# TWeber132/thesis-clip-nerf

Hardware: AMD Instinct MI355X
Metric: rendered rays/sec (64 samples/ray) at 1/2/4/8 MI355X; RGB L1 vs ref (higher is better)
Workload: dtype f32

## Files before the change

### thesis_clip_nerf_amd/csrc/field_eval_split16_impl.h

```cpp
#include <hip/hip_runtime.h>

#include "mvnerf_kernels.h"
#include "mvnerf_launch.h"
#include "mvnerf_math.h"
#include "mvnerf_mfma.h"

#ifndef MVS16_F16
#error "include through field_eval_split16.hip / field_eval_split16h.hip"
#endif
#if MVS16_F16
#define MVS16_BYTES packed_net_split16h_bytes
#define MVS16_PACK launch_pack_net_split16h
#define MVS16_SUPPORTS field_eval_split16h_supports
#define MVS16_LAUNCH_FN launch_field_eval_split16h
#define MVS16_KERNEL field_eval_split16h_kernel
#define MVS16_PACK_KERNEL pack_net_split16h_kernel
#else
#define MVS16_BYTES packed_net_split16_bytes
#define MVS16_PACK launch_pack_net_split16
#define MVS16_SUPPORTS field_eval_split16_supports
#define MVS16_LAUNCH_FN launch_field_eval_split16
#define MVS16_KERNEL field_eval_split16_kernel
#define MVS16_PACK_KERNEL pack_net_split16_kernel
#endif

namespace mvnerf {

namespace {

using bf16x8 = __attribute__((ext_vector_type(8))) __bf16;
using f16x8 = __attribute__((ext_vector_type(8))) _Float16;
using f16x2 = __attribute__((ext_vector_type(2))) _Float16;
using f32x2 = __attribute__((ext_vector_type(2))) float;
using u32x4 = __attribute__((ext_vector_type(4))) unsigned int;

constexpr int kS16SlotChunks = 24;
constexpr int kS16L0Pe = 2, kS16L0Feat = 8, kS16Hidden = 48;
constexpr int kS16Steps = kS16L0Pe + kS16L0Feat + kS16Hidden;
constexpr int kS16Chunks = kS16Steps * kS16SlotChunks;
constexpr int kChunkElems16 = 512;

__host__ __device__ constexpr int s16_pe_row(int g, int e) {
    return g < 3 ? 20 * g + e : (e < 12 ? 20 * (e >> 2) + 2 * (8 + ((e >> 1) & 1)) + (e & 1) : (e < 15 ? 120 + (e - 12) : -1));
}

__global__ void MVS16_PACK_KERNEL(const float* __restrict__ src, unsigned short* __restrict__ dst) {
    const int idx = blockIdx.x * blockDim.x + threadIdx.x;
    if (idx >= kS16Chunks * kChunkElems16) return;
    const int chunk = idx / kChunkElems16, lane = (idx % kChunkElems16) / 8, jj = idx % 8;
    const int i = lane & 15, g = lane >> 4;
    const int ks = chunk / kS16SlotChunks, rb = (chunk % kS16SlotChunks) / 3, piece = chunk % 3;
    float val = 0.0f;
    if (ks < kS16L0Pe) {
        const int row = s16_pe_row(g, 8 * ks + jj);
        if (row >= 0) val = src[kKerasW0 + row * kHidden + 16 * rb + i];
    } else if (ks < kS16L0Pe + kS16L0Feat) {
        const int row = 123 + 32 * (ks - kS16L0Pe) + 8 * g + jj;
        val = src[kKerasW0 + row * kHidden + 16 * rb + i];
    } else {
        const int q = ks - kS16L0Pe - kS16L0Feat, layer = q / 4, t = q % 4;
        const int f = 32 * t + (jj < 4 ? 4 * g + jj : 16 + 4 * g + (jj - 4));
        const int wsrc = kKerasBlocks + (layer / 2) * kKerasBlockStride + (layer % 2) * (kHidden * kHidden + kHidden);
        val = src[wsrc + f * kHidden + 16 * rb + i];
    }
#if MVS16_F16
    const float tw = val * 64.0f;
    const _Float16 a0 = (_Float16)tw;
    const _Float16 a1 = (_Float16)(tw - (float)a0);
    const _Float16 a0s = (_Float16)((float)a0 * 0.015625f);
    const _Float16 pc = piece == 0 ? a0 : (piece == 1 ? a0s : a1);
    dst[idx] = __builtin_bit_cast(unsigned short, pc);
#else
    const __bf16 p1 = (__bf16)val;
    const float r1 = val - (float)p1;
    const __bf16 p2 = (__bf16)r1;
    const float r2 = r1 - (float)p2;
    const __bf16 p3 = (__bf16)r2;
    const __bf16 pc = piece == 0 ? p1 : (piece == 1 ? p2 : p3);
    dst[idx] = __builtin_bit_cast(unsigned short, pc);
#endif
}

__device__ __forceinline__ f32x4 mfma1632(u32x4 a, u32x4 b, f32x4 c) {
#if MVS16_F16
    return __builtin_amdgcn_mfma_f32_16x16x32_f16(__builtin_bit_cast(f16x8, a), __builtin_bit_cast(f16x8, b), c, 0, 0, 0);
#else
    return __builtin_amdgcn_mfma_f32_16x16x32_bf16(__builtin_bit_cast(bf16x8, a), __builtin_bit_cast(bf16x8, b), c, 0, 0, 0);
#endif
}

struct B16 {
    u32x4 p1, p2, p3;
};

template <bool kRelu>
__device__ __forceinline__ void cut_pair(float v0, float v1, int q, B16& b) {
    if (kRelu) {
        const int i0 = __builtin_bit_cast(int, v0), i1 = __builtin_bit_cast(int, v1);
        v0 = __builtin_bit_cast(float, i0 > 0 ? i0 : 0);
        v1 = __builtin_bit_cast(float, i1 > 0 ? i1 : 0);
    }
#if MVS16_F16
    const f32x2 t = {v0 * 0.015625f, v1 * 0.015625f};
    const unsigned h = __builtin_bit_cast(unsigned, __builtin_convertvector(t, f16x2));
    float r0, r1;
    asm("v_fma_mix_f32 %0, %1, %2, %3 op_sel_hi:[1,0,0]" : "=v"(r0) : "v"(h), "s"(-64.0f), "v"(v0));
    asm("v_fma_mix_f32 %0, %1, %2, %3 op_sel:[1,0,0] op_sel_hi:[1,0,0]" : "=v"(r1) : "v"(h), "s"(-64.0f), "v"(v1));
    const f32x2 r = {r0, r1};
    b.p1[q] = h;
    b.p3[q] = __builtin_bit_cast(unsigned, __builtin_convertvector(r, f16x2));
#else
    const float r0 = v0 - __builtin_bit_cast(float, __builtin_bit_cast(unsigned, v0) & 0xffff0000u);
    const float r1 = v1 - __builtin_bit_cast(float, __builtin_bit_cast(unsigned, v1) & 0xffff0000u);
    const float s0 = r0 - __builtin_bit_cast(float, __builtin_bit_cast(unsigned, r0) & 0xffff0000u);
    const float s1 = r1 - __builtin_bit_cast(float, __builtin_bit_cast(unsigned, r1) & 0xffff0000u);
    b.p1[q] = __builtin_amdgcn_perm(__builtin_bit_cast(unsigned, v1), __builtin_bit_cast(unsigned, v0), 0x07060302u);
    b.p2[q] = __builtin_amdgcn_perm(__builtin_bit_cast(unsigned, r1), __builtin_bit_cast(unsigned, r0), 0x07060302u);
    b.p3[q] = __builtin_amdgcn_perm(__builtin_bit_cast(unsigned, s1), __builtin_bit_cast(unsigned, s0), 0x07060302u);
#endif
}

__device__ __forceinline__ void pin_pieces(B16& b, int q) {
#if MVS16_F16
    unsigned u1 = b.p1[q], u3 = b.p3[q];
    asm volatile("" : "+v"(u1), "+v"(u3));
    b.p1[q] = u1;
    b.p3[q] = u3;
#else
    unsigned u1 = b.p1[q], u2 = b.p2[q], u3 = b.p3[q];
    asm volatile("" : "+v"(u1), "+v"(u2), "+v"(u3));
    b.p1[q] = u1;
    b.p2[q] = u2;
    b.p3[q] = u3;
#endif
}

template <bool kRelu>
__device__ __forceinline__ void cut8(const float (&v)[8], B16& b) {
#pragma unroll
    for (int q = 0; q < 4; ++q) cut_pair<kRelu>(v[2 * q], v[2 * q + 1], q, b);
}

constexpr int kR16Slots = 3, kR16SlotF4 = kS16SlotChunks * 64;
constexpr int kS16PerView = kS16Hidden / 2;
constexpr int kS16MaxPositions = 512;

struct Ring16 {
    const f32x4* w;
    f32x4* base;
    int c;
    int p, P;
    const int* table;
    int start_pf;
    int tid, wave;
    u32x4 a0[3];
};

__device__ __forceinline__ int ring16_start_chunk(int p, int V, int l0_units) {
    const int per_view = l0_units + kS16PerView;
    if (p < per_view * V) {
        const int q = p % per_view;
        return (q < kS16L0Pe ? q : (q < l0_units ? q : kS16L0Pe + kS16L0Feat + (q - l0_units))) * kS16SlotChunks;
    }
    return (kS16L0Pe + kS16L0Feat + kS16PerView + (p - per_view * V)) * kS16SlotChunks;
}

__device__ __forceinline__ void ring16_dma(const Ring16& r, int start_chunk, int slot) {
    const f32x4* src = r.w + (long)start_chunk * 64 + r.tid;
    f32x4* dst = r.base + slot * kR16SlotF4 + 64 * r.wave;
#pragma unroll
    for (int i = 0; i < 3; ++i)
        __builtin_amdgcn_global_load_lds((const __attribute__((address_space(1))) void*)(src + 512 * i),
                                         (__attribute__((address_space(3))) void*)(dst + 512 * i), 16, 0, 0);
}

__device__ __forceinline__ void ring16_fetch(Ring16& r) {
    int slot = r.c + 2;
    slot = slot >= kR16Slots ? slot - kR16Slots : slot;
    ring16_dma(r, r.start_pf, slot);
    int pp = r.p + 3;
    pp = pp >= r.P ? pp - r.P : pp;
    r.start_pf = r.table[pp];
}

__device__ __forceinline__ const f32x4* ring16_cur(const Ring16& r) { return r.base + r.c * kR16SlotF4; }
__device__ __forceinline__ const f32x4* ring16_nxt(const Ring16& r) { return r.base + (r.c + 1 == kR16Slots ? 0 : r.c + 1) * kR16SlotF4; }

__device__ __forceinline__ void ring16_next(Ring16& r) {
    asm volatile("s_waitcnt vmcnt(0) lgkmcnt(0)\n\ts_barrier" ::: "memory");
    r.c = r.c + 1 == kR16Slots ? 0 : r.c + 1;
    r.p = r.p + 1 == r.P ? 0 : r.p + 1;
}

__device__ __forceinline__ int perm_f4(int rb, int g) {
    return ((g & 1) * 64 + (rb >> 1) * 16 + 4 * (2 * (rb & 1) + (g >> 1))) >> 2;
}

template <bool kAdd>
__device__ __forceinline__ void apply_bias_row(f32x4 (&row)[2], const f32x4& bv) {
#pragma unroll
    for (int cb = 0; cb < 2; ++cb)
#pragma unroll
        for (int c = 0; c < 4; ++c) {
            if (kAdd) {
                float r = row[cb][c];
                asm("v_add_f32_e32 %0, %1, %2" : "=v"(r) : "v"(r), "v"(bv[c]));
                row[cb][c] = r;
            } else {
                row[cb][c] = bv[c];
            }
        }
}

template <bool kRelu, int kMode, bool kTailAdd>
__device__ __forceinline__ void kstep16(Ring16& ring, int lane, int g, const B16 (&b)[2], const float (&nv)[2][8], B16 (&bn)[2], f32x4 (&acc)[8][2],
                                        f32x4 (&in)[8][2], const float* __restrict__ tail_bias) {
    const f32x4* cur = ring16_cur(ring) + lane;
    const f32x4* nxt = ring16_nxt(ring) + lane;
    u32x4 a[3] = {ring.a0[0], ring.a0[1], ring.a0[2]};
    f32x4 bv = {0.0f, 0.0f, 0.0f, 0.0f};
    int glane = (g & 1) * 16 + (g >> 1);
    if (kMode == 4) asm volatile("" : "+v"(glane));
    const f32x4* tail_rows = reinterpret_cast<const f32x4*>(tail_bias) + glane;
#pragma unroll
    for (int rb = 0; rb < 8; ++rb) {
        u32x4 an[3];
#pragma unroll
        for (int q = 0; q < 3; ++q) an[q] = __builtin_bit_cast(u32x4, rb < 7 ? cur[((rb + 1) * 3 + q) * 64] : nxt[q * 64]);
        if (kMode == 1) cut_pair<kRelu>(nv[rb >> 2][2 * (rb & 3)], nv[rb >> 2][2 * (rb & 3) + 1], rb & 3, bn[rb >> 2]);
        if (kMode == 4 && tail_bias) {
            const f32x4 bv_new = tail_rows[(rb >> 1) * 4 + 2 * (rb & 1)];
            if (rb > 0) apply_bias_row<kTailAdd>(in[rb - 1], bv);
            bv = bv_new;
        }
#if MVS16_F16
#pragma unroll
        for (int cb = 0; cb < 2; ++cb) acc[rb][cb] = mfma1632(a[1], b[cb].p3, acc[rb][cb]);
#pragma unroll
        for (int cb = 0; cb < 2; ++cb) acc[rb][cb] = mfma1632(a[2], b[cb].p1, acc[rb][cb]);
#pragma unroll
        for (int cb = 0; cb < 2; ++cb) acc[rb][cb] = mfma1632(a[0], b[cb].p1, acc[rb][cb]);
#else
#pragma unroll
        for (int cb = 0; cb < 2; ++cb) acc[rb][cb] = mfma1632(a[2], b[cb].p1, acc[rb][cb]);
#pragma unroll
        for (int cb = 0; cb < 2; ++cb) acc[rb][cb] = mfma1632(a[1], b[cb].p2, acc[rb][cb]);
#pragma unroll
        for (int cb = 0; cb < 2; ++cb) acc[rb][cb] = mfma1632(a[0], b[cb].p3, acc[rb][cb]);
#pragma unroll
        for (int cb = 0; cb < 2; ++cb) acc[rb][cb] = mfma1632(a[1], b[cb].p1, acc[rb][cb]);
#pragma unroll
        for (int cb = 0; cb < 2; ++cb) acc[rb][cb] = mfma1632(a[0], b[cb].p2, acc[rb][cb]);
#pragma unroll
        for (int cb = 0; cb < 2; ++cb) acc[rb][cb] = mfma1632(a[0], b[cb].p1, acc[rb][cb]);
#endif
        __builtin_amdgcn_sched_group_barrier(0x008, 1, 0);
        __builtin_amdgcn_sched_group_barrier(0x100, kMode == 4 ? 4 : 3, 0);
#pragma unroll
        for (int m = 0; m < (MVS16_F16 ? 5 : 11); ++m) {
            if (kMode == 1) __builtin_amdgcn_sched_group_barrier(0x002, MVS16_F16 ? 2 : 1, 0);
            if (kMode == 4) __builtin_amdgcn_sched_group_barrier(0x002, MVS16_F16 ? 2 : 1, 0);
            __builtin_amdgcn_sched_group_barrier(0x008, 1, 0);
        }
        if (kMode == 1) __builtin_amdgcn_sched_group_barrier(0x002, MVS16_F16 ? 3 : 2, 0);
        __builtin_amdgcn_sched_barrier(0);
        if (rb == 0) {
            ring16_fetch(ring);
            __builtin_amdgcn_sched_barrier(0);
        }
#pragma unroll
        for (int q = 0; q < 3; ++q) a[q] = an[q];
    }
#pragma unroll
    for (int q = 0; q < 3; ++q) ring.a0[q] = a[q];
    if (kMode == 4 && tail_bias) apply_bias_row<kTailAdd>(in[7], bv);
    if (kMode == 1) {
#pragma unroll
        for (int cb = 0; cb < 2; ++cb)
#pragma unroll
            for (int q = 0; q < 4; ++q) {
                pin_pieces(bn[cb], q);
            }
    }
}

__device__ __forceinline__ void first_operand_s16(const f32x4 (&in)[8][2], B16 (&b)[2]) {
#pragma unroll
    for (int cb = 0; cb < 2; ++cb) {
        const float v8[8] = {in[0][cb][0], in[0][cb][1], in[0][cb][2], in[0][cb][3], in[1][cb][0], in[1][cb][1], in[1][cb][2], in[1][cb][3]};
        cut8<true>(v8, b[cb]);
    }
}

template <bool kTailAdd>
__device__ __forceinline__ void dense128_s16_plain(Ring16& ring, int lane, int g, f32x4 (&in)[8][2], f32x4 (&acc)[8][2], const float* __restrict__ tail_bias) {
    B16 b[2], bn[2];
    first_operand_s16(in, b);
#pragma unroll
    for (int t = 0; t < 4; ++t) {
        float nv[2][8];
#pragma unroll
        for (int cb = 0; cb < 2; ++cb)
#pragma unroll
            for (int q = 0; q < 8; ++q) nv[cb][q] = t < 3 ? in[2 * (t + 1) + (q >> 2)][cb][q & 3] : 0.0f;
        if (t < 3) kstep16<true, 1, false>(ring, lane, g, b, nv, bn, acc, in, nullptr);
        else kstep16<true, 4, kTailAdd>(ring, lane, g, b, nv, bn, acc, in, tail_bias);
        b[0] = bn[0];
        b[1] = bn[1];
        ring16_next(ring);
    }
}

template <bool kAdd>
__device__ __forceinline__ void bias16(const float* __restrict__ bperm, int g, f32x4 (&acc)[8][2]) {
    const f32x4* p = reinterpret_cast<const f32x4*>(bperm);
#pragma unroll
    for (int rb = 0; rb < 8; ++rb) {
        const f32x4 v = p[perm_f4(rb, g)];
#pragma unroll
        for (int cb = 0; cb < 2; ++cb)
#pragma unroll
            for (int c = 0; c < 4; ++c) {
                if (kAdd) {
                    float r = acc[rb][cb][c];
                    asm("v_add_f32_e32 %0, %1, %2" : "=v"(r) : "v"(r), "v"(v[c]));
                    acc[rb][cb][c] = r;
                } else {
                    acc[rb][cb][c] = v[c];
                }
            }
    }
}

constexpr int kS16StageRowBytes = 256;

__device__ __forceinline__ void store_tl16(float* __restrict__ base, long tile, int n, int g, const f32x4 (&x)[8][2]) {
    const __amdgpu_buffer_rsrc_t rsrc = __builtin_amdgcn_make_buffer_rsrc(base, 0, 0xFFFFFFFF, 0x00020000);
    const int voff = (4 * g * 32 + n) * 4;
    const int tile_off = (int)((unsigned)tile * 16384u);
#pragma unroll
    for (int rb = 0; rb < 8; ++rb)
#pragma unroll
        for (int i = 0; i < 4; ++i)
#pragma unroll
            for (int cb = 0; cb < 2; ++cb) {
                const float val = x[rb][cb][i];
                __builtin_amdgcn_raw_buffer_store_b32(__builtin_bit_cast(unsigned int, val), rsrc, voff + (i * 32 + 16 * cb) * 4,
                                                      tile_off + rb * 2048, kStashAux);
            }
}

struct SampleGeo {
    long g;
    int ray, sidx, b;
    float wx, wy, wz;
    bool valid;
};

template <bool kMultiView, bool kProj, bool kAux, bool kStash>
__global__ __launch_bounds__(512, 2) void MVS16_KERNEL(FieldParams p, const f32x4* __restrict__ wsplit) {
    constexpr int kW = 8;
    extern __shared__ __attribute__((aligned(16))) unsigned char smem_s16[];
    constexpr int kRingBytes = kR16Slots * kR16SlotF4 * 16;
    const int tid = threadIdx.x, lane = tid & 63, n = lane & 15, g = lane >> 4;
    const int wave = __builtin_amdgcn_readfirstlane(tid >> 6);
    unsigned char* stage = smem_s16 + kRingBytes + wave * (32 * kS16StageRowBytes);
    float* net = reinterpret_cast<float*>(smem_s16 + kRingBytes + kW * 32 * kS16StageRowBytes) - kPackB0;
    for (int i = tid; i < kPackBr + 8 - kPackB0; i += 64 * kW) net[kPackB0 + i] = p.net[kPackB0 + i];
    int* table = reinterpret_cast<int*>(smem_s16 + kRingBytes + kW * 32 * kS16StageRowBytes + (kPackBr + 8 - kPackB0) * 4);
    float* wr_plain = reinterpret_cast<float*>(table + kS16MaxPositions);
    for (int i = tid; i < 512; i += 64 * kW) wr_plain[i] = p.net[kPackWrPlain + i];

    Ring16 ring;
    ring.w = wsplit;
    ring.base = reinterpret_cast<f32x4*>(smem_s16);
    ring.c = 0;
    ring.p = 0;
    const int l0_units = kProj ? kS16L0Pe : kS16L0Pe + kS16L0Feat;
    ring.P = (l0_units + kS16PerView) * p.V + kS16PerView;
    for (int i = tid; i < ring.P; i += 64 * kW) table[i] = ring16_start_chunk(i, p.V, l0_units);
    ring.table = table;
    __syncthreads();
    ring.tid = tid;
    ring.wave = wave;
    ring16_dma(ring, table[0], 0);
    ring16_dma(ring, table[1], 1);
    ring.start_pf = table[2];
    asm volatile("s_waitcnt vmcnt(0)" ::: "memory");
    __syncthreads();
#pragma unroll
    for (int q = 0; q < 3; ++q) ring.a0[q] = __builtin_bit_cast(u32x4, ring16_cur(ring)[q * 64 + lane]);

    const long n_groups = (p.n_tiles + kW - 1) / kW;
    for (long grp = blockIdx.x; grp < n_groups; grp += gridDim.x) {
        long tile = grp * kW + wave;
        const bool tile_ok = tile < p.n_tiles;
        if (!tile_ok) tile = p.n_tiles - 1;
        int pS = p.S, pR = p.R, pH = p.H, pW = p.W, gl = g, nl = n;
        asm volatile("" : "+s"(pS), "+s"(pR), "+s"(pH), "+s"(pW));
        asm volatile("" : "+v"(gl), "+v"(nl));
        SampleGeo sg[2];
#pragma unroll
        for (int cb = 0; cb < 2; ++cb) {
            long gi = tile * 32 + 16 * cb + nl;
            sg[cb].valid = tile_ok && gi < p.total;
            if (gi >= p.total) gi = p.total - 1;
            sg[cb].g = gi;
            const int ray = (int)((unsigned)gi / (unsigned)pS);
            sg[cb].ray = ray;
            sg[cb].sidx = (int)gi - ray * pS;
            sg[cb].b = (int)((unsigned)ray / (unsigned)pR);
            const float ox = p.rays_o[3 * ray + 0], oy = p.rays_o[3 * ray + 1], oz = p.rays_o[3 * ray + 2];
            const float dx = p.rays_d[3 * ray + 0], dy = p.rays_d[3 * ray + 1], dz = p.rays_d[3 * ray + 2];
            const float zz = p.z[gi];
            sg[cb].wx = ox + zz * dx;
            sg[cb].wy = oy + zz * dy;
            sg[cb].wz = oz + zz * dz;
        }

        f32x4 x[8][2], hid[8][2];
        f32x4 xsum[kMultiView ? 8 : 1][2];

        const int n_views = (kMultiView || !(kAux || kStash)) ? p.V : 1;
        for (int v = 0; v < n_views; ++v) {
            int tl[2];
            float ax[2], ay[2];
            long vrow[2];
            float pe[2][16];
#pragma unroll
            for (int cb = 0; cb < 2; ++cb) {
                const int bv = sg[cb].b * p.V + v;
                const float* E = p.einv + 16 * bv;
                float cam[4];
#pragma unroll
                for (int r = 0; r < 4; ++r) cam[r] = row_dot4(E, r, sg[cb].wx, sg[cb].wy, sg[cb].wz, 1.0f);
                float pxl, pyl;
                pixel_from_cam(p.k4 + 16 * bv, cam, &pxl, &pyl);
                const Taps tp = bilinear_taps(pxl, pyl, pH, pW);
                tl[cb] = (bv * pH + tp.y0) * pW + tp.x0;
                ax[cb] = tp.ax;
                ay[cb] = tp.ay;
                vrow[cb] = ((long)bv * pR + (sg[cb].ray - sg[cb].b * pR)) * pS + sg[cb].sidx;
                if (kAux && sg[cb].valid && gl == 0) {
                    if (p.tap_idx) {
                        int4 t4 = make_int4(tl[cb], tl[cb] + 1, tl[cb] + pW, tl[cb] + pW + 1);
                        *reinterpret_cast<int4*>(p.tap_idx + 4 * vrow[cb]) = t4;
                    }
                    if (p.pix) {
                        p.pix[2 * vrow[cb] + 0] = pxl;
                        p.pix[2 * vrow[cb] + 1] = pyl;
                    }
                }
                {
                    const f32x4* seed = reinterpret_cast<const f32x4*>(p.dir_bias + 128 * ((long)bv * pR + (sg[cb].ray - sg[cb].b * pR)));
#pragma unroll
                    for (int rb = 0; rb < 8; ++rb) x[rb][cb] = seed[perm_f4(rb, gl)];
                }
                {
                    const float cd = gl == 0 ? cam[0] : (gl == 1 ? cam[1] : cam[2]);
                    const float a0 = (gl < 3 ? cd : cam[0]) * 3.14159274101257324f;
                    const float a1 = (gl < 3 ? cd : cam[1]) * 3.14159274101257324f;
                    const float a2 = cam[2] * 3.14159274101257324f;
                    float s0, c0, s1, c1, s2, c2;
                    sincos_f32(a0 * (gl < 3 ? 1.0f : 256.0f), &s0, &c0);
                    sincos_f32(a1 * (gl < 3 ? 32.0f : 256.0f), &s1, &c1);
                    sincos_f32(a2 * 256.0f, &s2, &c2);
                    auto dbl = [](float& sk, float& ck) {
                        const float t2 = sk + sk;
                        const float cn = fmaf(-t2, sk, 1.0f);
                        sk = t2 * ck;
                        ck = cn;
                    };
                    float va[16], vb[16];
                    {
                        float sk = s0, ck = c0;
                        va[0] = sk; va[1] = ck;
#pragma unroll
                        for (int k = 1; k < 5; ++k) { dbl(sk, ck); va[2 * k] = sk; va[2 * k + 1] = ck; }
                        sk = s1; ck = c1;
                        va[10] = sk; va[11] = ck;
#pragma unroll
                        for (int k = 6; k < 8; ++k) { dbl(sk, ck); va[2 * k] = sk; va[2 * k + 1] = ck; }
                    }
                    {
                        float sk = s0, ck = c0;
                        vb[0] = sk; vb[1] = ck; dbl(sk, ck); vb[2] = sk; vb[3] = ck;
                        sk = s1; ck = c1;
                        vb[4] = sk; vb[5] = ck; dbl(sk, ck); vb[6] = sk; vb[7] = ck;
                        sk = s2; ck = c2;
                        vb[8] = sk; vb[9] = ck; dbl(sk, ck); vb[10] = sk; vb[11] = ck;
                        const float* img = p.images + 3 * (long)tl[cb];
#pragma unroll
                        for (int c = 0; c < 3; ++c) {
                            const float a = img[c] * 2.0f - 1.0f, bq = img[3 + c] * 2.0f - 1.0f;
                            const float cq = img[3 * pW + c] * 2.0f - 1.0f, dq = img[3 * pW + 3 + c] * 2.0f - 1.0f;
                            vb[12 + c] = bilerp(a, bq, cq, dq, tp.ax, tp.ay);
                        }
                        vb[15] = 0.0f;
                    }
#pragma unroll
                    for (int e = 0; e < 16; ++e) pe[cb][e] = gl < 3 ? va[e] : vb[e];
                }
            }

            {
                B16 bq[2], bqn[2];
#pragma unroll
                for (int cb = 0; cb < 2; ++cb) {
                    const float v8[8] = {pe[cb][0], pe[cb][1], pe[cb][2], pe[cb][3], pe[cb][4], pe[cb][5], pe[cb][6], pe[cb][7]};
                    cut8<false>(v8, bq[cb]);
                }
                float nv[2][8];
#pragma unroll
                for (int cb = 0; cb < 2; ++cb)
#pragma unroll
                    for (int q = 0; q < 8; ++q) nv[cb][q] = pe[cb][8 + q];
                kstep16<false, 1, false>(ring, lane, g, bq, nv, bqn, x, x, nullptr);
                ring16_next(ring);
                kstep16<false, 0, false>(ring, lane, g, bqn, nv, bq, x, x, nullptr);
                ring16_next(ring);
            }

            asm volatile("" : "+v"(gl), "+v"(nl));
#pragma unroll
            for (int P = 0; P < (kProj ? 2 : 4); ++P) {
                asm volatile("s_waitcnt lgkmcnt(0)" ::: "memory");
                const f32x4* tbase = kProj ? reinterpret_cast<const f32x4*>(p.texel_table) + (nl >> 3) * 16 + (nl & 7) + P * 8
                                           : reinterpret_cast<const f32x4*>(p.features) + P * 16 + nl;
                const long row_f4 = kProj ? 32 : 64;
#pragma unroll
                for (int half = 0; half < 2; ++half) {
                    f32x4 tv[4][4];
                    float axs[4], ays[4];
#pragma unroll
                    for (int u = 0; u < 4; ++u) {
                        const int src = 4 * u + gl;
                        const int tls = __shfl(tl[half], src);
                        axs[u] = __shfl(ax[half], src);
                        ays[u] = __shfl(ay[half], src);
                        const f32x4* f = tbase + (long)tls * row_f4;
                        tv[u][0] = f[0];
                        tv[u][1] = f[row_f4];
                        tv[u][2] = f[(long)pW * row_f4];
                        tv[u][3] = f[(long)pW * row_f4 + row_f4];
                    }
                    __builtin_amdgcn_sched_barrier(0);
#pragma unroll
                    for (int u = 0; u < 4; ++u) {
                        const int src = 16 * half + 4 * u + gl;
                        f32x4 o;
#pragma unroll
                        for (int c = 0; c < 4; ++c) {
                            const float top = fmaf(axs[u], tv[u][1][c] - tv[u][0][c], tv[u][0][c]);
                            const float bot = fmaf(axs[u], tv[u][3][c] - tv[u][2][c], tv[u][2][c]);
                            o[c] = fmaf(ays[u], bot - top, top);
                        }
                        *reinterpret_cast<f32x4*>(stage + src * kS16StageRowBytes + ((nl ^ (src & 15)) << 4)) = o;
                    }
                }
                asm volatile("s_waitcnt lgkmcnt(0)" ::: "memory");
                if (kProj) {
#pragma unroll
                    for (int cb = 0; cb < 2; ++cb)
#pragma unroll
                        for (int rbl = 0; rbl < 4; ++rbl) {
                            const int row = 16 * cb + nl, chunk = 8 * (gl & 1) + 4 * (rbl >> 1) + 2 * (rbl & 1) + (gl >> 1);
                            const f32x4 t4 = *reinterpret_cast<const f32x4*>(stage + row * kS16StageRowBytes + ((chunk ^ (row & 15)) << 4));
#pragma unroll
                            for (int c = 0; c < 4; ++c) x[4 * P + rbl][cb][c] += t4[c];
                        }
                } else {
#pragma unroll
                    for (int s = 0; s < 2; ++s) {
                        B16 bq[2], bqn[2];
                        float nv[2][8];
#pragma unroll
                        for (int cb = 0; cb < 2; ++cb) {
                            const int row = 16 * cb + nl;
                            const f32x4 lo = *reinterpret_cast<const f32x4*>(stage + row * kS16StageRowBytes + (((8 * s + 2 * gl) ^ (row & 15)) << 4));
                            const f32x4 hi = *reinterpret_cast<const f32x4*>(stage + row * kS16StageRowBytes + (((8 * s + 2 * gl + 1) ^ (row & 15)) << 4));
                            const float b8[8] = {lo[0], lo[1], lo[2], lo[3], hi[0], hi[1], hi[2], hi[3]};
                            cut8<false>(b8, bq[cb]);
#pragma unroll
                            for (int q = 0; q < 8; ++q) nv[cb][q] = 0.0f;
                        }
                        kstep16<false, 0, false>(ring, lane, gl, bq, nv, bqn, x, x, nullptr);
                        ring16_next(ring);
                    }
                }
            }

            const long vslot = (long)p.B * p.V * p.R * p.S * 128;
            const long vtile = kMultiView ? ((long)(sg[0].b * p.V + v) * (p.n_tiles / p.B) + (tile - (long)sg[0].b * (p.n_tiles / p.B))) : tile;
            if (kStash && tile_ok) store_tl16(p.stash, vtile, n, g, x);
            auto store_acc16 = [&](float* base, const long (&rows)[2]) {
#pragma unroll
                for (int cb = 0; cb < 2; ++cb)
                    if (sg[cb].valid) {
                        float* e = base + 128 * rows[cb] + 4 * g;
#pragma unroll
                        for (int rb = 0; rb < 8; ++rb) *reinterpret_cast<f32x4*>(e + 16 * rb) = x[rb][cb];
                    }
            };
            if (kAux && p.acts_view) store_acc16(p.acts_view, vrow);
            bias16<false>(net + kPackBHidden, g, hid);
#pragma unroll 1
            for (int bi = 0; bi < 3; ++bi) {
                const float* bias1 = net + kPackBHidden + 256 * bi;
                if (bi > 0) bias16<false>(bias1, g, hid);
                dense128_s16_plain<true>(ring, lane, g, x, hid, nullptr);
                if (kStash && tile_ok) store_tl16(p.stash + (1 + 2 * bi) * p.stash_stride, vtile, n, g, hid);
                bias16<true>(bias1 + 128, g, x);
                dense128_s16_plain<false>(ring, lane, g, hid, x, nullptr);
                if (kStash && tile_ok && bi < 2) store_tl16(p.stash + (2 + 2 * bi) * p.stash_stride, vtile, n, g, x);
                if (kAux && p.acts_view) store_acc16(p.acts_view + (bi + 1) * vslot, vrow);
            }
            if (kMultiView) {
#pragma unroll
                for (int rb = 0; rb < 8; ++rb)
#pragma unroll
                    for (int cb = 0; cb < 2; ++cb) xsum[rb][cb] = (v == 0) ? x[rb][cb] : xsum[rb][cb] + x[rb][cb];
            }
        }
        if (kMultiView) {
            const float nvw = (float)p.V;
#pragma unroll
            for (int rb = 0; rb < 8; ++rb)
#pragma unroll
                for (int cb = 0; cb < 2; ++cb) x[rb][cb] = xsum[rb][cb] / nvw;
        }

        long grow[2];
        bool gvalid[2];
        {
            int ne = n;
            asm volatile("" : "+v"(ne));
#pragma unroll
            for (int cb = 0; cb < 2; ++cb) {
                long gi = tile * 32 + 16 * cb + ne;
                gvalid[cb] = tile_ok && gi < p.total;
                grow[cb] = gi >= p.total ? p.total - 1 : gi;
            }
        }
        auto store_fused16 = [&](float* base) {
#pragma unroll
            for (int cb = 0; cb < 2; ++cb)
                if (gvalid[cb]) {
                    float* e = base + 128 * grow[cb] + 4 * g;
#pragma unroll
                    for (int rb = 0; rb < 8; ++rb) *reinterpret_cast<f32x4*>(e + 16 * rb) = x[rb][cb];
                }
        };
        if (kAux && p.acts_fused) store_fused16(p.acts_fused);
        if (kStash && tile_ok) store_tl16(p.stash_fused, tile, n, g, x);
#pragma unroll 1
        for (int bi = 3; bi < 6; ++bi) {
            const float* bias1 = net + kPackBHidden + 256 * bi;
            bias16<false>(bias1, g, hid);
            dense128_s16_plain<true>(ring, lane, g, x, hid, nullptr);
            if (kStash && tile_ok) store_tl16(p.stash_fused + (1 + 2 * (bi - 3)) * p.stash_fused_stride, tile, n, g, hid);
            bias16<true>(bias1 + 128, g, x);
            dense128_s16_plain<false>(ring, lane, g, hid, x, nullptr);
            if (kStash && tile_ok) store_tl16(p.stash_fused + (2 + 2 * (bi - 3)) * p.stash_fused_stride, tile, n, g, x);
            if (kAux && p.acts_fused) store_fused16(p.acts_fused + (long)(bi - 2) * p.total * 128);
        }
        if (kAux && p.embedding) store_fused16(p.embedding);

        {
            float o[2][4] = {{0.0f, 0.0f, 0.0f, 0.0f}, {0.0f, 0.0f, 0.0f, 0.0f}};
            const f32x4* wr = reinterpret_cast<const f32x4*>(wr_plain) + 4 * g;
#pragma unroll
            for (int rb = 0; rb < 8; ++rb)
#pragma unroll
                for (int c = 0; c < 4; ++c) {
                    const f32x4 w4 = wr[16 * rb + c];
#pragma unroll
                    for (int cb = 0; cb < 2; ++cb) {
                        const float a = fmaxf(x[rb][cb][c], 0.0f);
#pragma unroll
                        for (int k = 0; k < 4; ++k) o[cb][k] = fmaf(a, w4[k], o[cb][k]);
                    }
                }
#pragma unroll
            for (int cb = 0; cb < 2; ++cb)
#pragma unroll
                for (int k = 0; k < 4; ++k) {
                    float t = o[cb][k];
                    t = t + __shfl_xor(t, 16);
                    t = t + __shfl_xor(t, 32);
                    o[cb][k] = t + net[kPackBr + k];
                }
            const int cbs = g & 1;
            const float o0 = cbs ? o[1][0] : o[0][0], o1 = cbs ? o[1][1] : o[0][1], o2 = cbs ? o[1][2] : o[0][2], o3 = cbs ? o[1][3] : o[0][3];
            const bool ok = cbs ? gvalid[1] : gvalid[0];
            const long gi = cbs ? grow[1] : grow[0];
            if (ok && g < 2) {
                f32x4 out;
                out[0] = sigmoid_f32(o0);
                out[1] = sigmoid_f32(o1);
                out[2] = sigmoid_f32(o2);
                out[3] = softplus_f32(o3);
                *reinterpret_cast<f32x4*>(p.rgbs + 4 * gi) = out;
            }
        }
    }
    asm volatile("s_waitcnt vmcnt(0)" ::: "memory");
}

}

size_t MVS16_BYTES() { return (size_t)kS16Chunks * 1024; }

hipError_t MVS16_PACK(const float* net_keras, void* packed_split16, hipStream_t st) {
    const int n = kS16Chunks * kChunkElems16;
    hipLaunchKernelGGL(MVS16_PACK_KERNEL, dim3((n + 255) / 256), dim3(256), 0, st, net_keras, static_cast<unsigned short*>(packed_split16));
    return hipGetLastError();
}

bool MVS16_SUPPORTS(const FieldParams& p) {
    if (p.stash && (p.tap_idx || p.pix || p.embedding || p.acts_view || p.acts_fused)) return false;
    const int n_pos = ((p.texel_table ? kS16L0Pe : kS16L0Pe + kS16L0Feat) + kS16PerView) * p.V + kS16PerView;
    return n_pos <= kS16MaxPositions;
}

hipError_t MVS16_LAUNCH_FN(const FieldParams& p, const void* packed_split16, hipStream_t stream) {
    static DeviceSetup setup;
    if (!MVS16_SUPPORTS(p)) return hipErrorInvalidValue;
    const int lds_bytes = kR16Slots * kR16SlotF4 * 16 + 8 * 32 * kS16StageRowBytes + (kPackBr + 8 - kPackB0) * 4 + kS16MaxPositions * 4 + 512 * 4;
    int cus = 0;
    hipError_t e = device_setup(setup, {{&MVS16_KERNEL<false, false, false, false>, lds_bytes}, {&MVS16_KERNEL<false, true, false, false>, lds_bytes},
                                        {&MVS16_KERNEL<true, false, false, false>, lds_bytes}, {&MVS16_KERNEL<true, true, false, false>, lds_bytes},
                                        {&MVS16_KERNEL<false, false, true, false>, lds_bytes}, {&MVS16_KERNEL<false, true, true, false>, lds_bytes},
                                        {&MVS16_KERNEL<true, false, true, false>, lds_bytes}, {&MVS16_KERNEL<true, true, true, false>, lds_bytes},
                                        {&MVS16_KERNEL<false, false, false, true>, lds_bytes}, {&MVS16_KERNEL<false, true, false, true>, lds_bytes},
                                        {&MVS16_KERNEL<true, false, false, true>, lds_bytes}, {&MVS16_KERNEL<true, true, false, true>, lds_bytes}}, &cus);
    if (e != hipSuccess) return e;
    if ((e = launch_dir_bias(p, stream)) != hipSuccess) return e;
    const bool mv = p.V > 1;
    const long n_groups = (p.n_tiles + 7) / 8;
    const long resident = (long)cus;
    const unsigned wgs = (unsigned)(n_groups < resident ? n_groups : resident);
    const f32x4* w = static_cast<const f32x4*>(packed_split16);
    const dim3 grid(wgs), block(512);
#define MVS16_LAUNCH(MV, PROJ, AUX, STASH) hipLaunchKernelGGL((MVS16_KERNEL<MV, PROJ, AUX, STASH>), grid, block, lds_bytes, stream, p, w)
    const bool aux = p.tap_idx || p.pix || p.embedding || p.acts_view || p.acts_fused;
    if (p.stash && p.V > 1 && ((long)p.R * p.S) % 32 != 0) return hipErrorInvalidValue;
    if (p.stash) {
        const int variant = (mv ? 2 : 0) + (p.texel_table ? 1 : 0);
        switch (variant) {
            case 0: MVS16_LAUNCH(false, false, false, true); break;
            case 1: MVS16_LAUNCH(false, true, false, true); break;
            case 2: MVS16_LAUNCH(true, false, false, true); break;
            default: MVS16_LAUNCH(true, true, false, true); break;
        }
        return hipGetLastError();
    }
    const int variant = (mv ? 4 : 0) + (p.texel_table ? 2 : 0) + (aux ? 1 : 0);
    switch (variant) {
        case 0: MVS16_LAUNCH(false, false, false, false); break;
        case 1: MVS16_LAUNCH(false, false, true, false); break;
        case 2: MVS16_LAUNCH(false, true, false, false); break;
        case 3: MVS16_LAUNCH(false, true, true, false); break;
        case 4: MVS16_LAUNCH(true, false, false, false); break;
        case 5: MVS16_LAUNCH(true, false, true, false); break;
        case 6: MVS16_LAUNCH(true, true, false, false); break;
        default: MVS16_LAUNCH(true, true, true, false); break;
    }
#undef MVS16_LAUNCH
    return hipGetLastError();
}

}
```

Before: 4.733 million.

## Fold hidden bias into MFMA init, byte-offset weight ring, and per-ray uniform geometry

Several changes land at once. The weight ring now uses byte offsets, rotated cur/nxt/fill slots and inline-asm global_load_lds with SGPR addresses, which removes per-fetch modulo and index arithmetic. The first MFMA of each hidden layer is seeded directly with bias rows instead of running a separate bias16 pass. When samples per ray is a multiple of 32, ray, camera and intrinsics values are treated as wave-uniform and loaded through scalar constant-address-space reads. This adds hand-written asm, wait-count encodings and a fast path that depends on tile alignment, so correctness and portability risk go up.

```diff
diff --git a/thesis_clip_nerf_amd/csrc/field_eval_split16_impl.h b/thesis_clip_nerf_amd/csrc/field_eval_split16_impl.h
--- a/thesis_clip_nerf_amd/csrc/field_eval_split16_impl.h
+++ b/thesis_clip_nerf_amd/csrc/field_eval_split16_impl.h
@@ -33,6 +33,7 @@
 using f16x2 = __attribute__((ext_vector_type(2))) _Float16;
 using f32x2 = __attribute__((ext_vector_type(2))) float;
 using u32x4 = __attribute__((ext_vector_type(4))) unsigned int;
+using cfloat = const __attribute__((address_space(4))) float;
 
 constexpr int kS16SlotChunks = 24;
 constexpr int kS16L0Pe = 2, kS16L0Feat = 8, kS16Hidden = 48;
@@ -147,12 +148,12 @@
 
 struct Ring16 {
     const f32x4* w;
-    f32x4* base;
-    int c;
-    int p, P;
+    unsigned char* lds;
+    int cur, nxt, fill;
     const int* table;
+    int pf4, P4;
     int start_pf;
-    int tid, wave;
+    int lane_off, wave_off;
     u32x4 a0[3];
 };
 
@@ -165,31 +166,30 @@
     return (kS16L0Pe + kS16L0Feat + kS16PerView + (p - per_view * V)) * kS16SlotChunks;
 }
 
-__device__ __forceinline__ void ring16_dma(const Ring16& r, int start_chunk, int slot) {
-    const f32x4* src = r.w + (long)start_chunk * 64 + r.tid;
-    f32x4* dst = r.base + slot * kR16SlotF4 + 64 * r.wave;
+__device__ __forceinline__ void ring16_dma(const Ring16& r, int start, int slot) {
+    const unsigned char* src = reinterpret_cast<const unsigned char*>(r.w) + (unsigned)start;
+    const int dst = (int)(unsigned long)(__attribute__((address_space(3))) unsigned char*)r.lds + slot + r.wave_off;
 #pragma unroll
     for (int i = 0; i < 3; ++i)
-        __builtin_amdgcn_global_load_lds((const __attribute__((address_space(1))) void*)(src + 512 * i),
-                                         (__attribute__((address_space(3))) void*)(dst + 512 * i), 16, 0, 0);
+        asm volatile("s_mov_b32 m0, %2\n\ts_nop 0\n\tglobal_load_lds_dwordx4 %0, %1" : : "v"(r.lane_off), "s"(src + 8192 * i), "s"(dst + 8192 * i) : "memory", "m0");
 }
 
 __device__ __forceinline__ void ring16_fetch(Ring16& r) {
-    int slot = r.c + 2;
-    slot = slot >= kR16Slots ? slot - kR16Slots : slot;
-    ring16_dma(r, r.start_pf, slot);
-    int pp = r.p + 3;
-    pp = pp >= r.P ? pp - r.P : pp;
-    r.start_pf = r.table[pp];
-}
-
-__device__ __forceinline__ const f32x4* ring16_cur(const Ring16& r) { return r.base + r.c * kR16SlotF4; }
-__device__ __forceinline__ const f32x4* ring16_nxt(const Ring16& r) { return r.base + (r.c + 1 == kR16Slots ? 0 : r.c + 1) * kR16SlotF4; }
+    ring16_dma(r, __builtin_amdgcn_readfirstlane(r.start_pf), r.fill);
+    r.start_pf = *reinterpret_cast<const int*>(reinterpret_cast<const unsigned char*>(r.table) + r.pf4);
+    r.pf4 = r.pf4 + 4 == r.P4 ? 0 : r.pf4 + 4;
+}
+
+__device__ __forceinline__ const f32x4* ring16_cur(const Ring16& r) { return reinterpret_cast<const f32x4*>(r.lds + r.cur); }
+__device__ __forceinline__ const f32x4* ring16_nxt(const Ring16& r) { return reinterpret_cast<const f32x4*>(r.lds + r.nxt); }
 
 __device__ __forceinline__ void ring16_next(Ring16& r) {
-    asm volatile("s_waitcnt vmcnt(0) lgkmcnt(0)\n\ts_barrier" ::: "memory");
-    r.c = r.c + 1 == kR16Slots ? 0 : r.c + 1;
-    r.p = r.p + 1 == r.P ? 0 : r.p + 1;
+    __builtin_amdgcn_s_waitcnt(0x0070);
+    asm volatile("s_barrier" ::: "memory");
+    const int done = r.cur;
+    r.cur = r.nxt;
+    r.nxt = r.fill;
+    r.fill = done;
 }
 
 __device__ __forceinline__ int perm_f4(int rb, int g) {
@@ -212,22 +212,27 @@
         }
 }
 
-template <bool kRelu, int kMode, bool kTailAdd>
+template <bool kRelu, int kMode, bool kTailAdd, bool kInit = false>
 __device__ __forceinline__ void kstep16(Ring16& ring, int lane, int g, const B16 (&b)[2], const float (&nv)[2][8], B16 (&bn)[2], f32x4 (&acc)[8][2],
-                                        f32x4 (&in)[8][2], const float* __restrict__ tail_bias) {
+                                        f32x4 (&in)[8][2], const float* __restrict__ tail_bias, const float* __restrict__ init_bias = nullptr,
+                                        f32x4 init0 = f32x4{0.0f, 0.0f, 0.0f, 0.0f}) {
     const f32x4* cur = ring16_cur(ring) + lane;
     const f32x4* nxt = ring16_nxt(ring) + lane;
     u32x4 a[3] = {ring.a0[0], ring.a0[1], ring.a0[2]};
     f32x4 bv = {0.0f, 0.0f, 0.0f, 0.0f};
     int glane = (g & 1) * 16 + (g >> 1);
-    if (kMode == 4) asm volatile("" : "+v"(glane));
+    if (kMode == 4 || kInit) asm volatile("" : "+v"(glane));
     const f32x4* tail_rows = reinterpret_cast<const f32x4*>(tail_bias) + glane;
+    const f32x4* init_rows = reinterpret_cast<const f32x4*>(init_bias) + glane;
+    f32x4 ci = init0;
 #pragma unroll
     for (int rb = 0; rb < 8; ++rb) {
         u32x4 an[3];
 #pragma unroll
         for (int q = 0; q < 3; ++q) an[q] = __builtin_bit_cast(u32x4, rb < 7 ? cur[((rb + 1) * 3 + q) * 64] : nxt[q * 64]);
         if (kMode == 1) cut_pair<kRelu>(nv[rb >> 2][2 * (rb & 3)], nv[rb >> 2][2 * (rb & 3) + 1], rb & 3, bn[rb >> 2]);
+        f32x4 cin = ci;
+        if (kInit && rb < 7) cin = init_rows[((rb + 1) >> 1) * 4 + 2 * ((rb + 1) & 1)];
         if (kMode == 4 && tail_bias) {
             const f32x4 bv_new = tail_rows[(rb >> 1) * 4 + 2 * (rb & 1)];
             if (rb > 0) apply_bias_row<kTailAdd>(in[rb - 1], bv);
@@ -235,14 +240,14 @@
         }
 #if MVS16_F16
 #pragma unroll
-        for (int cb = 0; cb < 2; ++cb) acc[rb][cb] = mfma1632(a[1], b[cb].p3, acc[rb][cb]);
+        for (int cb = 0; cb < 2; ++cb) acc[rb][cb] = mfma1632(a[1], b[cb].p3, kInit ? ci : acc[rb][cb]);
 #pragma unroll
         for (int cb = 0; cb < 2; ++cb) acc[rb][cb] = mfma1632(a[2], b[cb].p1, acc[rb][cb]);
 #pragma unroll
         for (int cb = 0; cb < 2; ++cb) acc[rb][cb] = mfma1632(a[0], b[cb].p1, acc[rb][cb]);
 #else
 #pragma unroll
-        for (int cb = 0; cb < 2; ++cb) acc[rb][cb] = mfma1632(a[2], b[cb].p1, acc[rb][cb]);
+        for (int cb = 0; cb < 2; ++cb) acc[rb][cb] = mfma1632(a[2], b[cb].p1, kInit ? ci : acc[rb][cb]);
 #pragma unroll
         for (int cb = 0; cb < 2; ++cb) acc[rb][cb] = mfma1632(a[1], b[cb].p2, acc[rb][cb]);
 #pragma unroll
@@ -255,7 +260,7 @@
         for (int cb = 0; cb < 2; ++cb) acc[rb][cb] = mfma1632(a[0], b[cb].p1, acc[rb][cb]);
 #endif
         __builtin_amdgcn_sched_group_barrier(0x008, 1, 0);
-        __builtin_amdgcn_sched_group_barrier(0x100, kMode == 4 ? 4 : 3, 0);
+        __builtin_amdgcn_sched_group_barrier(0x100, (kMode == 4 || kInit) ? 4 : 3, 0);
 #pragma unroll
         for (int m = 0; m < (MVS16_F16 ? 5 : 11); ++m) {
             if (kMode == 1) __builtin_amdgcn_sched_group_barrier(0x002, MVS16_F16 ? 2 : 1, 0);
@@ -265,11 +270,13 @@
         if (kMode == 1) __builtin_amdgcn_sched_group_barrier(0x002, MVS16_F16 ? 3 : 2, 0);
         __builtin_amdgcn_sched_barrier(0);
         if (rb == 0) {
+            asm volatile("" : "+v"(acc[0][0]), "+v"(acc[0][1]));
             ring16_fetch(ring);
             __builtin_amdgcn_sched_barrier(0);
         }
 #pragma unroll
         for (int q = 0; q < 3; ++q) a[q] = an[q];
+        ci = cin;
     }
 #pragma unroll
     for (int q = 0; q < 3; ++q) ring.a0[q] = a[q];
@@ -292,9 +299,12 @@
     }
 }
 
-template <bool kTailAdd>
-__device__ __forceinline__ void dense128_s16_plain(Ring16& ring, int lane, int g, f32x4 (&in)[8][2], f32x4 (&acc)[8][2], const float* __restrict__ tail_bias) {
+template <bool kTailAdd, bool kInit>
+__device__ __forceinline__ void dense128_s16_plain(Ring16& ring, int lane, int g, f32x4 (&in)[8][2], f32x4 (&acc)[8][2], const float* __restrict__ tail_bias,
+                                                   const float* __restrict__ init_bias = nullptr) {
     B16 b[2], bn[2];
+    f32x4 init0 = {0.0f, 0.0f, 0.0f, 0.0f};
+    if (kInit) init0 = reinterpret_cast<const f32x4*>(init_bias)[perm_f4(0, g)];
     first_operand_s16(in, b);
 #pragma unroll
     for (int t = 0; t < 4; ++t) {
@@ -303,7 +313,8 @@
         for (int cb = 0; cb < 2; ++cb)
 #pragma unroll
             for (int q = 0; q < 8; ++q) nv[cb][q] = t < 3 ? in[2 * (t + 1) + (q >> 2)][cb][q & 3] : 0.0f;
-        if (t < 3) kstep16<true, 1, false>(ring, lane, g, b, nv, bn, acc, in, nullptr);
+        if (t == 0 && kInit) kstep16<true, 1, false, true>(ring, lane, g, b, nv, bn, acc, in, nullptr, init_bias, init0);
+        else if (t < 3) kstep16<true, 1, false>(ring, lane, g, b, nv, bn, acc, in, nullptr);
         else kstep16<true, 4, kTailAdd>(ring, lane, g, b, nv, bn, acc, in, tail_bias);
         b[0] = bn[0];
         b[1] = bn[1];
@@ -313,10 +324,12 @@
 
 template <bool kAdd>
 __device__ __forceinline__ void bias16(const float* __restrict__ bperm, int g, f32x4 (&acc)[8][2]) {
-    const f32x4* p = reinterpret_cast<const f32x4*>(bperm);
+    int glane = (g & 1) * 16 + (g >> 1);
+    asm volatile("" : "+v"(glane));
+    const f32x4* p = reinterpret_cast<const f32x4*>(bperm) + glane;
 #pragma unroll
     for (int rb = 0; rb < 8; ++rb) {
-        const f32x4 v = p[perm_f4(rb, g)];
+        const f32x4 v = p[(rb >> 1) * 4 + 2 * (rb & 1)];
 #pragma unroll
         for (int cb = 0; cb < 2; ++cb)
 #pragma unroll
@@ -373,49 +386,76 @@
 
     Ring16 ring;
     ring.w = wsplit;
-    ring.base = reinterpret_cast<f32x4*>(smem_s16);
-    ring.c = 0;
-    ring.p = 0;
+    ring.lds = smem_s16;
+    ring.cur = 0;
+    ring.nxt = kR16SlotF4 * 16;
+    ring.fill = 2 * kR16SlotF4 * 16;
     const int l0_units = kProj ? kS16L0Pe : kS16L0Pe + kS16L0Feat;
-    ring.P = (l0_units + kS16PerView) * p.V + kS16PerView;
-    for (int i = tid; i < ring.P; i += 64 * kW) table[i] = ring16_start_chunk(i, p.V, l0_units);
+    const int n_pos = (l0_units + kS16PerView) * p.V + kS16PerView;
+    for (int i = tid; i < n_pos; i += 64 * kW) table[i] = ring16_start_chunk(i, p.V, l0_units) * 1024;
     ring.table = table;
+    ring.P4 = 4 * n_pos;
+    ring.pf4 = 4 * 3;
     __syncthreads();
-    ring.tid = tid;
-    ring.wave = wave;
-    ring16_dma(ring, table[0], 0);
-    ring16_dma(ring, table[1], 1);
+    ring.lane_off = 16 * tid;
+    ring.wave_off = 1024 * wave;
+    ring16_dma(ring, __builtin_amdgcn_readfirstlane(table[0]), ring.cur);
+    ring16_dma(ring, __builtin_amdgcn_readfirstlane(table[1]), ring.nxt);
     ring.start_pf = table[2];
     asm volatile("s_waitcnt vmcnt(0)" ::: "memory");
     __syncthreads();
 #pragma unroll
     for (int q = 0; q < 3; ++q) ring.a0[q] = __builtin_bit_cast(u32x4, ring16_cur(ring)[q * 64 + lane]);
 
-    const long n_groups = (p.n_tiles + kW - 1) / kW;
-    for (long grp = blockIdx.x; grp < n_groups; grp += gridDim.x) {
-        long tile = grp * kW + wave;
-        const bool tile_ok = tile < p.n_tiles;
-        if (!tile_ok) tile = p.n_tiles - 1;
+    const int n_tiles = (int)p.n_tiles, n_groups = (n_tiles + kW - 1) / kW;
+    for (int grp = blockIdx.x; grp < n_groups; grp += gridDim.x) {
+        const int own = grp * kW + wave;
+        const bool tile_ok = own < n_tiles;
+        const long tile = tile_ok ? own : n_tiles - 1;
         int pS = p.S, pR = p.R, pH = p.H, pW = p.W, gl = g, nl = n;
         asm volatile("" : "+s"(pS), "+s"(pR), "+s"(pH), "+s"(pW));
         asm volatile("" : "+v"(gl), "+v"(nl));
         SampleGeo sg[2];
-#pragma unroll
-        for (int cb = 0; cb < 2; ++cb) {
-            long gi = tile * 32 + 16 * cb + nl;
-            sg[cb].valid = tile_ok && gi < p.total;
-            if (gi >= p.total) gi = p.total - 1;
-            sg[cb].g = gi;
-            const int ray = (int)((unsigned)gi / (unsigned)pS);
-            sg[cb].ray = ray;
-            sg[cb].sidx = (int)gi - ray * pS;
-            sg[cb].b = (int)((unsigned)ray / (unsigned)pR);
-            const float ox = p.rays_o[3 * ray + 0], oy = p.rays_o[3 * ray + 1], oz = p.rays_o[3 * ray + 2];
-            const float dx = p.rays_d[3 * ray + 0], dy = p.rays_d[3 * ray + 1], dz = p.rays_d[3 * ray + 2];
-            const float zz = p.z[gi];
-            sg[cb].wx = ox + zz * dx;
-            sg[cb].wy = oy + zz * dy;
-            sg[cb].wz = oz + zz * dz;
+        const bool one_ray = (pS & 31) == 0;
+        if (one_ray) {
+            const unsigned first = (unsigned)tile * 32u;
+            const int ray = __builtin_amdgcn_readfirstlane((int)(first / (unsigned)pS));
+            const int b = __builtin_amdgcn_readfirstlane((int)((unsigned)ray / (unsigned)pR));
+            const int s0 = (int)first - ray * pS;
+            const cfloat* ro = (const cfloat*)(p.rays_o + 3 * ray);
+            const cfloat* rd = (const cfloat*)(p.rays_d + 3 * ray);
+            const float ox = ro[0], oy = ro[1], oz = ro[2], dx = rd[0], dy = rd[1], dz = rd[2];
+#pragma unroll
+            for (int cb = 0; cb < 2; ++cb) {
+                const long gi = (long)first + 16 * cb + nl;
+                sg[cb].valid = tile_ok;
+                sg[cb].g = gi;
+                sg[cb].ray = ray;
+                sg[cb].sidx = s0 + 16 * cb + nl;
+                sg[cb].b = b;
+                const float zz = p.z[gi];
+                sg[cb].wx = ox + zz * dx;
+                sg[cb].wy = oy + zz * dy;
+                sg[cb].wz = oz + zz * dz;
+            }
+        } else {
+#pragma unroll
+            for (int cb = 0; cb < 2; ++cb) {
+                long gi = tile * 32 + 16 * cb + nl;
+                sg[cb].valid = tile_ok && gi < p.total;
+                if (gi >= p.total) gi = p.total - 1;
+                sg[cb].g = gi;
+                const int ray = (int)((unsigned)gi / (unsigned)pS);
+                sg[cb].ray = ray;
+                sg[cb].sidx = (int)gi - ray * pS;
+                sg[cb].b = (int)((unsigned)ray / (unsigned)pR);
+                const float ox = p.rays_o[3 * ray + 0], oy = p.rays_o[3 * ray + 1], oz = p.rays_o[3 * ray + 2];
+                const float dx = p.rays_d[3 * ray + 0], dy = p.rays_d[3 * ray + 1], dz = p.rays_d[3 * ray + 2];
+                const float zz = p.z[gi];
+                sg[cb].wx = ox + zz * dx;
+                sg[cb].wy = oy + zz * dy;
+                sg[cb].wz = oz + zz * dz;
+            }
         }
 
         f32x4 x[8][2], hid[8][2];
@@ -423,6 +463,9 @@
 
         const int n_views = (kMultiView || !(kAux || kStash)) ? p.V : 1;
         for (int v = 0; v < n_views; ++v) {
+            asm volatile("" : "+s"(pS), "+s"(pR), "+s"(pH), "+s"(pW));
+#pragma unroll
+            for (int cb = 0; cb < 2; ++cb) asm volatile("" : "+v"(sg[cb].b), "+v"(sg[cb].ray), "+v"(sg[cb].sidx));
             int tl[2];
             float ax[2], ay[2];
             long vrow[2];
@@ -430,12 +473,31 @@
 #pragma unroll
             for (int cb = 0; cb < 2; ++cb) {
                 const int bv = sg[cb].b * p.V + v;
-                const float* E = p.einv + 16 * bv;
-                float cam[4];
-#pragma unroll
-                for (int r = 0; r < 4; ++r) cam[r] = row_dot4(E, r, sg[cb].wx, sg[cb].wy, sg[cb].wz, 1.0f);
-                float pxl, pyl;
-                pixel_from_cam(p.k4 + 16 * bv, cam, &pxl, &pyl);
+                float cam[4], pxl, pyl;
+                const f32x4* seed;
+                if (one_ray) {
+                    const int bu = __builtin_amdgcn_readfirstlane(sg[0].b), bvu = bu * p.V + v;
+                    const int rayu = __builtin_amdgcn_readfirstlane(sg[0].ray);
+                    const cfloat* Ec = (const cfloat*)(p.einv + 16 * bvu);
+                    const cfloat* Kc = (const cfloat*)(p.k4 + 16 * bvu);
+                    float E[16], K[12];
+#pragma unroll
+                    for (int i = 0; i < 16; ++i) E[i] = Ec[i];
+#pragma unroll
+                    for (int i = 0; i < 12; ++i) K[i] = Kc[i];
+#pragma unroll
+                    for (int r = 0; r < 4; ++r) cam[r] = row_dot4(E, r, sg[cb].wx, sg[cb].wy, sg[cb].wz, 1.0f);
+                    pixel_from_cam(K, cam, &pxl, &pyl);
+                    seed = reinterpret_cast<const f32x4*>(p.dir_bias + 128 * ((long)bvu * pR + (rayu - bu * pR)));
+                } else {
+                    const float* E = p.einv + 16 * bv;
+#pragma unroll
+                    for (int r = 0; r < 4; ++r) cam[r] = row_dot4(E, r, sg[cb].wx, sg[cb].wy, sg[cb].wz, 1.0f);
+                    pixel_from_cam(p.k4 + 16 * bv, cam, &pxl, &pyl);
+                    seed = reinterpret_cast<const f32x4*>(p.dir_bias + 128 * ((long)bv * pR + (sg[cb].ray - sg[cb].b * pR)));
+                }
+#pragma unroll
+                for (int rb = 0; rb < 8; ++rb) x[rb][cb] = seed[perm_f4(rb, gl)];
                 const Taps tp = bilinear_taps(pxl, pyl, pH, pW);
                 tl[cb] = (bv * pH + tp.y0) * pW + tp.x0;
                 ax[cb] = tp.ax;
@@ -450,11 +512,6 @@
                         p.pix[2 * vrow[cb] + 0] = pxl;
                         p.pix[2 * vrow[cb] + 1] = pyl;
                     }
-                }
-                {
-                    const f32x4* seed = reinterpret_cast<const f32x4*>(p.dir_bias + 128 * ((long)bv * pR + (sg[cb].ray - sg[cb].b * pR)));
-#pragma unroll
-                    for (int rb = 0; rb < 8; ++rb) x[rb][cb] = seed[perm_f4(rb, gl)];
                 }
                 {
                     const float cd = gl == 0 ? cam[0] : (gl == 1 ? cam[1] : cam[2]);
@@ -603,15 +660,13 @@
                     }
             };
             if (kAux && p.acts_view) store_acc16(p.acts_view, vrow);
-            bias16<false>(net + kPackBHidden, g, hid);
 #pragma unroll 1
             for (int bi = 0; bi < 3; ++bi) {
                 const float* bias1 = net + kPackBHidden + 256 * bi;
-                if (bi > 0) bias16<false>(bias1, g, hid);
-                dense128_s16_plain<true>(ring, lane, g, x, hid, nullptr);
+                dense128_s16_plain<true, true>(ring, lane, g, x, hid, nullptr, bias1);
                 if (kStash && tile_ok) store_tl16(p.stash + (1 + 2 * bi) * p.stash_stride, vtile, n, g, hid);
                 bias16<true>(bias1 + 128, g, x);
-                dense128_s16_plain<false>(ring, lane, g, hid, x, nullptr);
+                dense128_s16_plain<false, false>(ring, lane, g, hid, x, nullptr);
                 if (kStash && tile_ok && bi < 2) store_tl16(p.stash + (2 + 2 * bi) * p.stash_stride, vtile, n, g, x);
                 if (kAux && p.acts_view) store_acc16(p.acts_view + (bi + 1) * vslot, vrow);
             }
@@ -656,11 +711,10 @@
 #pragma unroll 1
         for (int bi = 3; bi < 6; ++bi) {
             const float* bias1 = net + kPackBHidden + 256 * bi;
-            bias16<false>(bias1, g, hid);
-            dense128_s16_plain<true>(ring, lane, g, x, hid, nullptr);
+            dense128_s16_plain<true, true>(ring, lane, g, x, hid, nullptr, bias1);
             if (kStash && tile_ok) store_tl16(p.stash_fused + (1 + 2 * (bi - 3)) * p.stash_fused_stride, tile, n, g, hid);
             bias16<true>(bias1 + 128, g, x);
-            dense128_s16_plain<false>(ring, lane, g, hid, x, nullptr);
+            dense128_s16_plain<false, false>(ring, lane, g, hid, x, nullptr);
             if (kStash && tile_ok) store_tl16(p.stash_fused + (2 + 2 * (bi - 3)) * p.stash_fused_stride, tile, n, g, x);
             if (kAux && p.acts_fused) store_fused16(p.acts_fused + (long)(bi - 2) * p.total * 128);
         }
```

After: 4.927 million, median of 6. 4.1% higher.
